# Aedelon/ProteinBERT-PyTorch-Replication

Hardware: AMD Instinct MI355X
Metric: sequences/sec (whole node) ProteinBERT pretrain L=512 at 1/2/4/8 MI355X (higher is better)
Workload: dtype bf16; 1 GPU; global_batch=2048, per_gpu_batch=2048, seq_len=512, parallelism=dp1, impl=hip, hip_graph=False

## Files before the change

### proteinbert_pytorch_replication_amd/ops/csrc/wgrad.hip

```cpp
#include "mfma.h"
#include <stdlib.h>

using namespace pbx;
typedef unsigned short bf16_t;

namespace {
constexpr int CH = 128;

constexpr int BM = 128;
constexpr int KS = 9;

__device__ __attribute__((aligned(16))) unsigned int g_zero16[4];
__device__ __attribute__((aligned(16))) unsigned int g_ones16[4] = {~0u, ~0u, ~0u, ~0u};

__device__ __forceinline__ void glds16(const void* src, unsigned char* lds_base) {
  const unsigned dst = __builtin_amdgcn_readfirstlane(
      (unsigned)(size_t)(__attribute__((address_space(3))) unsigned char*)lds_base);
  unsigned keep;
  asm volatile("s_mov_b32 %0, m0\n\ts_mov_b32 m0, %2\n\ts_nop 0\n\tglobal_load_lds_dwordx4 %1, off\n\ts_mov_b32 m0, %0"
               : "=&s"(keep)
               : "v"(src), "s"(dst)
               : "memory");
}

// ... 351 lines not shown
    sg.zero = opaque_addr(g_zero16);
    sg.ones = opaque_addr(g_ones16);
    sg.pos0 = tt0 * TBM;
    sg.L = L;
    sg.n0 = rows0 / 4;
    sg.n = rows0 / 4 + rows1 / 4;
    sg.w = w;
    sg.hal1 = hal1;
    sg.lane = lane;
    sg.lrow = lane >> 4;
    sg.lx = (unsigned)((lane & 15) ^ (((lane >> 4) & 3) << 2));
  }

  f32x16_t acc[KS];
#pragma unroll
  for (int k = 0; k < KS; ++k) acc[k] = zero16();
  const int hal = cv ? hal1 : hal0;
  const int colb = ct * 32 + tc;
  const int cvb = cv ? rows0 * 256 : 0;
  int boff[KS], boff4[KS];
#pragma unroll
  for (int k = 0; k < KS; ++k) {
    const int rb = hal + (KS / 2 - k) * d + 8 * h + q;
    boff[k] = cvb + swz256e(rb, colb);
    boff4[k] = cvb + swz256e(rb + 4, colb);
  }
  const int toff = (rows0 + rows1) * 256 + 8 * h * 8;
  if (nt > 0) {
    sg.all(smem);
    sg.next();
  }
  for (int it = 0; it < nt; ++it) {
    unsigned char* cur = smem + (it & 1) * buf_bytes;
    unsigned char* nxt = smem + ((it & 1) ^ 1) * buf_bytes;
    asm volatile("s_waitcnt vmcnt(0)" ::: "memory");
    __syncthreads();
    const int nn = it + 1 < nt ? sg.n : -1;
    constexpr int NS = (TBM / 16) * KS;
    static_assert(MAXET <= NS, "one DMA per step");
    bf16x8 fb[3], fa[2];
    unsigned tk[8];
    auto read_b = [&](int st) {
      const unsigned char* c = cur + (st / KS) * 4096;
      fb[st % 3] = cat_tr(lds_tr(c, boff[st % KS]), lds_tr(c, boff4[st % KS]));
    };
    auto read_tok = [&](int kb) {
      const unsigned* tp = reinterpret_cast<const unsigned*>(cur + toff + kb * 128);
#pragma unroll
      for (int j = 0; j < 8; ++j) tk[j] = tp[2 * j];
    };
    auto make_a = [&](int kb) {
      typedef __attribute__((ext_vector_type(4))) unsigned int u32x4;
      u32x4 o;
#pragma unroll
      for (int e = 0; e < 4; ++e)
        o[e] = (tk[2 * e] == (unsigned)r ? 0x3F80u : 0u) | (tk[2 * e + 1] == (unsigned)r ? 0x3F800000u : 0u);
      fa[kb & 1] = __builtin_bit_cast(bf16x8, o);
    };
    read_tok(0);
    make_a(0);
    read_b(0);
    read_b(1);
#pragma unroll
    for (int st = 0; st < NS; ++st) {
      const int kb = st / KS, k = st % KS;
      if (st + 2 < NS) read_b(st + 2);
      if (k == 3 && kb + 1 < TBM / 16) read_tok(kb + 1);
      if (k == 7 && kb + 1 < TBM / 16) make_a(kb + 1);
      __builtin_amdgcn_sched_barrier(0);
      if (st < MAXET) sg.issue(st, nn, nxt);
      acc[k] = mfma32(fa[kb & 1], fb[st % 3], acc[k]);
    }
    sg.next();
  }
#pragma unroll
  for (int k = 0; k < KS; ++k)
#pragma unroll
    for (int i = 0; i < 16; ++i) {
      const int v = (i & 3) + 8 * (i >> 2) + 4 * h;
      if (v < V) slab[((((size_t)blockIdx.x * 2 + cv) * KS + k) * V + v) * CH + ct * 32 + r] = acc[k][i];
    }
}

__global__ void __launch_bounds__(128) wgrad_tok_finish_kernel(const float* __restrict__ S, const float* __restrict__ E,
                                                               float* __restrict__ dw0, float* __restrict__ dw1,
                                                               float* __restrict__ db0, float* __restrict__ db1,
                                                               int V, const float* __restrict__ W0,
                                                               const float* __restrict__ W1, float* __restrict__ dEslab) {
  __shared__ float sv[KS * 32];
  const int c = blockIdx.x / CH, co = blockIdx.x % CH, ci = threadIdx.x;
  for (int i = threadIdx.x; i < KS * V; i += 128) {
    const int k = i / V, v = i % V;
    sv[k * 32 + v] = S[(((size_t)c * KS + k) * V + v) * CH + co];
  }
  __syncthreads();
  float o[KS];
#pragma unroll
  for (int k = 0; k < KS; ++k) o[k] = 0.f;
  for (int v = 0; v < V; ++v) {
    const float e = bfround(E[v * CH + ci]);
#pragma unroll
    for (int k = 0; k < KS; ++k) o[k] = fmaf(e, sv[k * 32 + v], o[k]);
  }
  float* dw = (c ? dw1 : dw0) + ((size_t)co * CH + ci) * KS;
#pragma unroll
  for (int k = 0; k < KS; ++k) dw[k] += o[k];
  if (ci == 0) {
    float s = 0.f;
    for (int v = 0; v < V; ++v) s += sv[(KS / 2) * 32 + v];
    (c ? db1 : db0)[co] += s;
  }
  if (dEslab != nullptr) {
    const float* wr = (c ? W1 : W0) + ((size_t)co * CH + ci) * KS;
    float wk[KS];
#pragma unroll
    for (int k = 0; k < KS; ++k) wk[k] = bfround(wr[k]);
    for (int v = 0; v < V; ++v) {
      float a = 0.f;
#pragma unroll
      for (int k = 0; k < KS; ++k) a = fmaf(wk[k], sv[k * 32 + v], a);
      dEslab[((size_t)blockIdx.x * V + v) * CH + ci] = a;
    }
  }
}

bool wgrad_tok_attr_set = false;
}

extern "C" int pbx_colsum_add(const float* src, int rows, int cols, float* dst, const float* scale, hipStream_t st);
extern "C" int pbx_colsum_set(const float* src, int rows, int cols, float* dst, const float* scale, hipStream_t st);

PBX_EXPORT int pbx_wgrad_tok_rows(int B, int L) {
  constexpr int cap = 256;
  const long NT = (long)B * ((L + TBM - 1) / TBM);
  return (int)(NT < cap ? NT : cap);
}

PBX_EXPORT int pbx_wgrad_tok(const void* tok, const void* dy0, const void* dy1, const float* E, float* slab, float* S,
                             float* dw0, float* dw1, float* db0, float* db1, int B, int L, int dil1, int V,
                             const float* W0, const float* W1, float* dE, float* dEslab, hipStream_t st) {
  if (V < 1 || V > 32 || dil1 < 1 || (L & 1) || B < 1 || L < 1) return (int)hipErrorInvalidValue;
  if ((dE == nullptr) != (W0 == nullptr) || (dE == nullptr) != (W1 == nullptr) || (dE == nullptr) != (dEslab == nullptr))
    return (int)hipErrorInvalidValue;
  const int buf = (2 * TBM + 8 + 8 * dil1) * 256 + 1024;
  if (2 * buf > 163840) return (int)hipErrorInvalidValue;
  if (!wgrad_tok_attr_set) {
    (void)hipFuncSetAttribute((const void*)wgrad_tok_kernel, hipFuncAttributeMaxDynamicSharedMemorySize, 163840);
    wgrad_tok_attr_set = true;
  }
  const int R = pbx_wgrad_tok_rows(B, L);
  hipLaunchKernelGGL(wgrad_tok_kernel, dim3(R), dim3(512), 2 * buf, st, (const long long*)tok, (const bf16_t*)dy0,
                     (const bf16_t*)dy1, slab, B, L, dil1, R, V, buf);
  const int cols = 2 * KS * V * CH;
  int rc = pbx_colsum_set(slab, R, cols, S, nullptr, st);
  if (rc != 0) return rc;
  hipLaunchKernelGGL(wgrad_tok_finish_kernel, dim3(2 * CH), dim3(128), 0, st, S, E, dw0, dw1, db0, db1, V, W0, W1,
                     dEslab);
  if (dE == nullptr) return pbx_launch_status();
  rc = pbx_launch_status();
  if (rc != 0) return rc;
  return pbx_colsum_add(dEslab, 2 * CH, V * CH, dE, nullptr, st);
}
```

### proteinbert_pytorch_replication_amd/ops/local_track.py

```python
from __future__ import annotations

import os
from typing import List, Dict, Optional, Tuple

import torch

from . import _lib, streams
from ..train.arena import notify_grads_ready
from ..utils.determinism import fused_deterministic
from .global_track import bf16_of

CH = 128
PB = 32
LN_EPS = 1e-5


BM1 = 128
def attn_pool_supported(NJ: int) -> bool:
    return NJ in (256, 512)


def conv_tile(L: int) -> int:
    return BM1

# ... 81 lines not shown
        _lib.call("pbx_wgrad2x", dy0.data_ptr(), _p(dy1), x.data_ptr(), slab.data_ptr(), bslab.data_ptr(),
                  dw0.data_ptr(), _p(dw1), db0.data_ptr(), _p(db1), B, L, dil, nconv, R, xlo, xhi, _lib.stream_ptr(dev))
    else:
        _lib.call("pbx_wgrad2", dy0.data_ptr(), _p(dy1), x.data_ptr(), slab.data_ptr(), bslab.data_ptr(),
                  dw0.data_ptr(), _p(dw1), db0.data_ptr(), _p(db1), B, L, dil, nconv, R, _lib.stream_ptr(dev))
    return [slab, bslab]


WGRAD_TOK = True
EMBED_FOLD = True
EMBED_GATHER = True


CONV_TOK = os.environ.get("PBX_CONV_TOK", "1") == "1"


def conv_tok_ok(B: int, L: int, KS: int, dil: int, V: int) -> bool:
    return CONV_TOK and bool(_lib.lib().pbx_conv_fwd_tok_ok(B, L, KS, dil, V))


def conv_tok_tables(wpn: torch.Tensor, wpw: torch.Tensor, emb_b: torch.Tensor) -> torch.Tensor:
    V = emb_b.shape[0]
    tab = torch.empty((2, 2, 9, V + 1, CH // 2), dtype=torch.float32, device=emb_b.device)
    _lib.call("pbx_conv_tok_tables", wpn.data_ptr(), wpw.data_ptr(), emb_b.data_ptr(), tab.data_ptr(), V,
              _lib.stream_ptr(emb_b.device))
    return tab


def conv_fwd_first(tok, emb_b, wpn, wpw, bn, bw, gb, pre_n, pre_w, s1, KS, dil, stream, tok_tab=None):
    B, L = tok.shape
    V = emb_b.shape[0]
    if conv_tok_ok(B, L, KS, dil, V):
        T1, bm1 = L // 4, 4
        st1 = torch.empty((B, T1, 2), dtype=torch.float32, device=tok.device)
        if tok_tab is None:
            tok_tab = conv_tok_tables(wpn, wpw, emb_b)
        _lib.call("pbx_conv_fwd_tok", tok.data_ptr(), emb_b.data_ptr(), tok_tab.data_ptr(), bn.data_ptr(),
                  bw.data_ptr(), gb.data_ptr(), _p(pre_n), _p(pre_w), s1.data_ptr(), st1.data_ptr(), B, L, KS, dil, V,
                  stream)
    else:
        T1, bm1 = (L + BM1 - 1) // BM1, BM1
        st1 = torch.empty((B, T1, 2), dtype=torch.float32, device=tok.device)
        _lib.call("pbx_conv_fwd3t", tok.data_ptr(), emb_b.data_ptr(), wpn.data_ptr(), wpw.data_ptr(), bn.data_ptr(),
                  bw.data_ptr(), gb.data_ptr(), _p(pre_n), _p(pre_w), s1.data_ptr(), st1.data_ptr(), B, L, KS, dil,
                  stream)
    return st1, T1, bm1


def wgrad_tok_ok(tok: Optional[torch.Tensor], emb: Optional[torch.Tensor], L: int, KS: int) -> bool:
    return (WGRAD_TOK and tok is not None and emb is not None and KS == 9 and L % 2 == 0
            and emb.shape[0] <= 32 and emb.shape[1] == CH and tok.dtype == torch.int64 and tok.is_contiguous())


def _wgrad_tok(dy0: torch.Tensor, dy1: torch.Tensor, tok: torch.Tensor, emb: torch.Tensor, dil: int, B: int, L: int,
               outs, demb=None):
    dev = dy0.device
    V = emb.shape[0]
    R = _lib.lib().pbx_wgrad_tok_rows(B, L)
    slab = torch.empty((R, 2, 9, V, CH), dtype=torch.float32, device=dev)
    S = torch.empty((2, 9, V, CH), dtype=torch.float32, device=dev)
    e = emb.detach().float().contiguous()
    (dw0, db0), (dw1, db1) = outs
    w0 = w1 = dE = dEslab = None
    if demb is not None:
        w0, w1 = (w.detach().float().contiguous() for w in demb[:2])
        dE = demb[2]
        dEslab = torch.empty((2 * CH, V, CH), dtype=torch.float32, device=dev)
    _lib.call("pbx_wgrad_tok", tok.data_ptr(), dy0.data_ptr(), dy1.data_ptr(), e.data_ptr(), slab.data_ptr(),
              S.data_ptr(), dw0.data_ptr(), dw1.data_ptr(), db0.data_ptr(), db1.data_ptr(), B, L, dil, V,
              _p(w0), _p(w1), _p(dE), _p(dEslab), _lib.stream_ptr(dev))
    return [slab, S, e, w0, w1, dEslab]


def embed_fold_bwd(tok, emb, ds1, gdn, gdw, dpn, dpw, wn, ww, stream):
    B, L = tok.shape
    dE, direct = _grad_dst(emb, emb.shape)
    slab = None
    if fused_deterministic():
        slab = torch.empty((_lib.lib().pbx_embed_bwd_groups(B * L), emb.shape[0], CH), dtype=torch.float32,
                           device=ds1.device)
    _lib.call("pbx_embed_dpre", tok.data_ptr(), ds1.data_ptr(), gdn.data_ptr(), gdw.data_ptr(), dpn.data_ptr(),
              dpw.data_ptr(), dE.data_ptr(), B * L, emb.shape[0], _p(slab), stream)
    return (wn, ww, dE), direct


class LocalBlockFn(torch.autograd.Function):

    @staticmethod
    def forward(ctx, x, gb, wn, bn, ww, bw, g1, be1, wl, bl, g2, be2, wv_bf16, dil: int, packed=None,
                tail: bool = False, cp=None, tok=None, emb=None, emb_grad: bool = False, tok_tab=None):
        params = (wn, bn, ww, bw, g1, be1, wl, bl, g2, be2)
        ctx.cp = cp
        if cp is not None:
            g1, be1, g2, be2 = (cp.rows(t) for t in (g1, be1, g2, be2))
        if x is None:
            if not (emb_grad and tok is not None and emb is not None and cp is None):
                raise ValueError("x may be None only for the folded first block (emb_grad with tok / emb)")
            B, L = tok.shape
            xt = torch.empty((B, L, CH), dtype=torch.bfloat16, device=tok.device)
        else:
            B, L, C = x.shape
            assert C == CH and x.dtype == torch.bfloat16 and x.is_contiguous()
            xt = x
        NJ = wv_bf16.shape[0]
        if not attn_pool_supported(NJ):
            raise NotImplementedError(f"HIP attention pool: H * value_dim = {NJ} (kernels built for 256 / 512)")
        KS = wn.shape[2]
        dev = xt.device
        stream = _lib.stream_ptr(dev)
        T1, bm1 = (L + BM1 - 1) // BM1, BM1
        T2 = (L + PB - 1) // PB
        if packed is not None:
            wpn, wtn, wpw, wtw = packed
        else:
            wpn, wtn = pack_conv(wn)
            wpw, wtw = pack_conv(ww)
        wl_b = bf16_of(wl)
        need_bwd = any(ctx.needs_input_grad)
        pre_n = torch.empty_like(xt) if need_bwd else None
        pre_w = torch.empty_like(xt) if need_bwd else None
        s1 = torch.empty_like(xt)
        gb = gb.detach().float().contiguous()
        from_tok = x is None or (cp is None and tok is not None and emb is not None and tok.dtype == torch.int64
                                 and tok.is_contiguous() and tuple(tok.shape) == (B, L) and emb.shape[1] == CH
                                 and conv_tok_ok(B, L, KS, dil, emb.shape[0]))
        if from_tok:
            x_ext, hlo = x, 0
            emb_b = bf16_of(emb)
            st1, T1, bm1 = conv_fwd_first(tok, emb_b, wpn, wpw, bn, bw, gb, pre_n, pre_w, s1, KS, dil, stream,
                                          tok_tab)
        elif cp is None:
            x_ext, hlo = x, 0
            st1 = torch.empty((B, T1, 2), dtype=torch.float32, device=dev)
            conv_fwd(x, wpn, wpw, bn, bw, gb, pre_n, pre_w, s1, st1, B, L, KS, dil, stream)
        else:
            x_ext, hlo = cp.halo_rows(x), cp.halo
            st1 = torch.empty((B, T1, 2), dtype=torch.float32, device=dev)
            conv_fwd(x_ext, wpn, wpw, bn, bw, gb, pre_n, pre_w, s1, st1, B, L, KS, dil, stream, hlo, hlo)
            cp.fix_stats(st1, BM1)
        pre_l = torch.empty_like(xt) if need_bwd else None
        s2 = torch.empty_like(xt)
        st2 = torch.empty((B, T2, 2), dtype=torch.float32, device=dev)
        _lib.call("pbx_ln_linear_fwd", s1.data_ptr(), st1.data_ptr(), T1, bm1, g1.data_ptr(), be1.data_ptr(),
                  wl_b.data_ptr(), bl.data_ptr(), _p(pre_l), s2.data_ptr(), st2.data_ptr(), B, L, LN_EPS, stream)
        if cp is not None:
            cp.fix_stats(st2, PB)
        h2 = torch.empty_like(xt)
        TV = (L + 31) // 32
        vpart = torch.empty((B, TV, NJ), dtype=torch.float32, device=dev)
        _lib.call("pbx_pool_fwd", s2.data_ptr(), st2.data_ptr(), g2.data_ptr(), be2.data_ptr(), wv_bf16.data_ptr(),
                  h2.data_ptr(), vpart.data_ptr(), B, L, NJ, LN_EPS, stream)
        ctx.save_for_backward(x_ext, pre_n, pre_w, s1, st1, pre_l, s2, st2, h2, wtn, wtw, wl_b, wv_bf16, g1, be1, g2,
                              be2)
        ctx.hlo = hlo
        ctx.tok = (tok, emb) if cp is None and wgrad_tok_ok(tok, emb, L, KS) else None
        ctx.emb_grad = bool(emb_grad)
        if ctx.emb_grad and (ctx.tok is None or (x is not None and x.requires_grad)):
            raise ValueError("emb_grad needs a token-embedding input without autograd history (wgrad_tok_ok)")
        ctx.meta = (B, L, KS, dil, T1, T2, NJ)
        ctx.bm1 = bm1
        ctx.tail = bool(tail) and WGRAD_TAIL_FULL
        ctx.set_materialize_grads(False)
        ctx.params = params
        return h2, vpart

    @staticmethod
    def backward(ctx, dh2, dvpart):
        streams.wait_ready(dvpart, dh2)
        (x_ext, pre_n, pre_w, s1, st1, pre_l, s2, st2, h2, wtn, wtw, wl_b, wv_bf16, g1, be1, g2,
         be2) = ctx.saved_tensors
        cp, hlo = ctx.cp, ctx.hlo
        x = s1
        B, L, KS, dil, T1, T2, NJ = ctx.meta
        bm1 = ctx.bm1
        dev = x.device
        stream = _lib.stream_ptr(dev)
        params = ctx.params
        dsts = [_grad_dst(p, p.shape) for p in params]
        (dwn, _), (dbn, _), (dww, _), (dbw, _), (dg1, _), (dbe1, _), (dwl, _), (dbl, _), (dg2, _), (dbe2, _) = dsts
        if cp is not None:
            dg1, dbe1, dg2, dbe2 = (cp.rows(t) for t in (dg1, dbe1, dg2, dbe2))
        dh2 = None if dh2 is None else dh2.to(torch.bfloat16).contiguous()
        TA = (L + 31) // 32
        if dvpart is None:
            dv, dv_tiles = torch.zeros((B, NJ), dtype=torch.float32, device=dev), 1
        elif dvpart.dim() == 3 and (dvpart.shape[1] == 1 or dvpart.stride(1) == 0):
            dv, dv_tiles = dvpart[:, 0, :].float().contiguous(), 1
        else:
            dv, dv_tiles = dvpart.float().contiguous(), TA
        dh2t = torch.empty_like(x)
        sums2 = torch.empty((B, TA, 2), dtype=torch.float32, device=dev)
        consts = torch.empty((B, 8), dtype=torch.float32, device=dev)
        dgb = torch.empty((B, CH), dtype=torch.float32, device=dev)
        _lib.call("pbx_pool_bwd", h2.data_ptr(), g2.data_ptr(), be2.data_ptr(), _p(dh2), dv.data_ptr(), dv_tiles,
                  wv_bf16.data_ptr(), dh2t.data_ptr(), sums2.data_ptr(), B, L, NJ, stream)
        if cp is not None:
            cp.fix_sums(sums2)
        dh1 = torch.empty_like(x)
        TS1 = (L + 1) // 2
        sums1 = torch.empty((B, TS1, 2), dtype=torch.float32, device=dev)
        det = int(fused_deterministic())
        late_fold = LN2_LATE_FOLD and streams.ENABLED and dev.type == "cuda" and dsts[6][1] and dsts[7][1]
        if late_fold:
            rows = _lib.lib().pbx_ln2_bwd_slab_rows(B, L, det)
            fslab = torch.empty(rows * (CH * CH + CH), dtype=torch.float32, device=dev)
            slab_args = (fslab.data_ptr(), rows)
        else:
            slab_args = dwl_slab(dev)
        _lib.call("pbx_ln2_linear_bwd", dh2t.data_ptr(), s2.data_ptr(), st2.data_ptr(), sums2.data_ptr(), TA,
                  g2.data_ptr(), pre_l.data_ptr(), s1.data_ptr(), st1.data_ptr(), T1, bm1, g1.data_ptr(),
                  be1.data_ptr(), wl_b.data_ptr(), consts.data_ptr(), dh1.data_ptr(), sums1.data_ptr(),
                  dg2.data_ptr(), dbe2.data_ptr(), dg1.data_ptr(), dbe1.data_ptr(), dwl.data_ptr(), dbl.data_ptr(),
                  dgb.data_ptr(), B, L, LN_EPS, *slab_args, det, int(not late_fold), 0, stream)
        if late_fold:
            def fold(slab=fslab, rows=rows, dwl=dwl, dbl=dbl):
                st = _lib.stream_ptr(dev)
                _lib.call("pbx_colsum_add2", slab.data_ptr(), CH * CH, dwl.data_ptr(), slab[rows * CH * CH:].data_ptr(),
                          CH, dbl.data_ptr(), rows, st)
            streams.launch(dev, fold, keep=[fslab], name="wgrad")
        dx = None if ctx.emb_grad else torch.empty_like(x)
        dpn = torch.empty_like(x)
        dpw = torch.empty_like(x)
        if cp is not None:
            cp.fix_sums(sums1)
        fin = (DGRAD_FIN and cp is None and not ctx.emb_grad and KS == 9 and dev.type == "cuda"
               and not fused_deterministic())

        def dgb_ready():
            if ctx.tail and INPUT_BWD_EARLY and streams.ENABLED and dev.type == "cuda":
                streams.fork(dev, "ann")

        if not fin:
            ds1 = torch.empty_like(x)
            _lib.call("pbx_ln1_finalize", dh1.data_ptr(), s1.data_ptr(), st1.data_ptr(), T1, bm1, sums1.data_ptr(),
                      TS1, g1.data_ptr(), ds1.data_ptr(), dgb.data_ptr(), B, L, LN_EPS, int(fused_deterministic()),
                      stream)
            if cp is not None:
                cp.all_reduce_(dgb)
            dgb_ready()
        demb = None
        if fin:
            conv_dgrad_fin(dh1, s1, st1, T1, bm1, sums1, TS1, g1, pre_n, pre_w, wtn, wtw, dx, dpn, dpw, dgb, B, L,
                           KS, dil, stream)
            dgb_ready()
        elif ctx.emb_grad:
            demb, dE_direct = embed_fold_bwd(*ctx.tok, ds1, pre_n, pre_w, dpn, dpw, params[0], params[2], stream)
            dE = demb[2]
        elif cp is None:
            conv_dgrad(ds1, pre_n, pre_w, wtn, wtw, dx, dpn, dpw, B, L, KS, dil, stream)
        else:
            conv_dgrad(*cp.halo_rows_many(ds1, pre_n, pre_w), wtn, wtw, dx, dpn, dpw, B, L,
                       KS, dil, stream, hlo, hlo)
        if ctx.tok is not None:
            tok, emb = ctx.tok
            wg = lambda: _wgrad_tok(dpn, dpw, tok, emb, dil, B, L, [(dwn, dbn), (dww, dbw)], demb)
            keep = [dpn, dpw, tok] + ([demb[2]] if demb is not None else [])
        else:
            wg = lambda: _wgrad(dpn, dpw, x_ext, KS, dil, 2, B, L, [(dwn, dbn), (dww, dbw)],
                                ctx.tail and streams.ENABLED, hlo, hlo)
            keep = [dpn, dpw, x_ext]
        direct = [p for p, (_, d) in zip(params, dsts) if d]
        if demb is not None and dE_direct:
            direct.append(ctx.tok[1])
        if all(dsts[i][1] for i in (0, 1, 2, 3)) and (demb is None or dE_direct) and streams.ENABLED:
            streams.launch(dev, wg, keep=keep, name="wgrad")
        else:
            wg()
        if direct:
            notify_grads_ready(direct)
        pgrads = [None if d else g for (g, d) in dsts]
        gemb = dE if demb is not None and not dE_direct else None
        return (dx, dgb, *pgrads, None, None, None, None, None, None, gemb, None, None)


def embed_tokens(tokens: torch.Tensor, weight: torch.Tensor) -> torch.Tensor:
    B, L = tokens.shape
    tok = tokens.contiguous()
    out = torch.empty((B, L, weight.shape[1]), dtype=torch.bfloat16, device=tokens.device)
    _lib.call("pbx_embed_fwd", tok.data_ptr(), weight.detach().contiguous().data_ptr(), out.data_ptr(), B * L,
              _lib.stream_ptr(tokens.device))
    return out


class EmbedFn(torch.autograd.Function):

    @staticmethod
    def forward(ctx, tokens, weight):
        B, L = tokens.shape
        V, C = weight.shape
        assert C == CH and V <= 32
        tok = tokens.contiguous()
        out = torch.empty((B, L, C), dtype=torch.bfloat16, device=tokens.device)
        _lib.call("pbx_embed_fwd", tok.data_ptr(), weight.detach().contiguous().data_ptr(), out.data_ptr(), B * L,
                  _lib.stream_ptr(tokens.device))
        ctx.save_for_backward(tok)
        ctx.V = V
        return out

    @staticmethod
    def backward(ctx, dout):
        (tok,) = ctx.saved_tensors
        dE = torch.zeros((ctx.V, CH), dtype=torch.float32, device=tok.device)
        d = dout.to(torch.bfloat16).contiguous()
        slab = None
        if fused_deterministic():
            g = _lib.lib().pbx_embed_bwd_groups(tok.numel())
            slab = torch.empty((g, ctx.V, CH), dtype=torch.float32, device=tok.device)
        _lib.call("pbx_embed_bwd", tok.data_ptr(), d.data_ptr(), dE.data_ptr(), tok.numel(), ctx.V, _lib.ptr(slab),
                  _lib.stream_ptr(tok.device))
        return None, dE


def _wv_bf16(att) -> torch.Tensor:
    Wv = att.Wv
    if isinstance(Wv, torch.nn.Parameter) and Wv.requires_grad:
        return att.value_weight_cat().t().to(torch.bfloat16).contiguous()
    key = (Wv.data_ptr(), Wv._version, Wv.device)
    cached = getattr(att, "_pbx_wv_cache", None)
    if cached is None or cached[0] != key:
        cached = (key, att.value_weight_cat().t().to(torch.bfloat16).contiguous())
        att._pbx_wv_cache = cached
    return cached[1]


def conv_images(wn: torch.Tensor, ww: torch.Tensor):
    KS = wn.shape[2]
    imgs = tuple(torch.empty((KS, CH, CH), dtype=torch.bfloat16, device=wn.device) for _ in range(4))
    return imgs, [(0, wn.detach(), imgs[0], imgs[1], KS, 0), (0, ww.detach(), imgs[2], imgs[3], KS, 0)]


def local_block(x: torch.Tensor, gb: torch.Tensor, blk, packed=None, tail: bool = False,
                cp=None, tok=None, emb=None, emb_grad: bool = False, tok_tab=None) -> Tuple[torch.Tensor, torch.Tensor]:
    att = blk.global_attention_layer
    wv = _wv_bf16(att)
    nc = blk.local_narrow_conv_layer[0]
    wc = blk.local_wide_conv_layer[0]
# ... 5 lines not shown
```

### proteinbert_pytorch_replication_amd/ops/paper_track.py

```python
from __future__ import annotations

import math

import torch

from . import _lib, streams
from ..train.arena import notify_grads_ready
from .gemm import gemm as _gemm
from .global_track import (BF16, F32, _Grads, _UNIT_LOSS_GRAD, bf16_of, go_head_backward, go_head_forward,
                           loss_total, mm32, addmm_into)
from .local_track import (CH, conv_dgrad, conv_fwd, conv_tile, dwl_slab, pack_conv, _grad_dst, _wgrad,
                          _wgrad_tok, embed_fold_bwd, wgrad_tok_ok)


def group_colsum(t: torch.Tensor) -> torch.Tensor:
    G, R, C = t.shape
    if t.device.type != "cuda":
        return t.sum(dim=1)
    t = t.contiguous()
    out = torch.empty((G, C), dtype=F32, device=t.device)
    _lib.call("pbx_group_colsum", t.data_ptr(), G, R, C, out.data_ptr(), _lib.stream_ptr(t.device))
    return out


def _sg_ws(B: int, G: int, H: int, K: int, dev) -> torch.Tensor:
    return torch.empty(_lib.lib().pbx_sg_query_ws(B, G, H, K), dtype=torch.float32, device=dev)

PAPER_ATTN = "fused"
FUSED_CHUNK_F = 256
FUSED_BWD_WAVES = 8

LN_EPS = 1e-5
TR = 32


class PaperBlockFn(torch.autograd.Function):

    @staticmethod
    def forward(ctx, x, gb, g, wn, bn, ww, bw, g1, be1, wl, bl, g2, be2, Wq, Wk, Wv, mask, dil: int, packed=None,
                tok=None, emb=None, emb_grad: bool = False, cp=None):
        from .paper_attention import KEY_DIM, VALUE_DIM, _nsplit
        params = (wn, bn, ww, bw, g1, be1, wl, bl, g2, be2, Wq, Wk, Wv)
        B, L, C = x.shape
        assert C == CH and x.dtype == BF16 and x.is_contiguous()
        assert g1.shape == (CH,), "paper semantics: LayerNorm affine is [C]"
        H, _, K = Wk.shape
        VD = Wv.shape[2]
        assert K == KEY_DIM and VD == VALUE_DIM
        KS = wn.shape[2]
        dev = x.device
        stream = _lib.stream_ptr(dev)
        BM1 = conv_tile(L)
        T1 = (L + BM1 - 1) // BM1
        if packed is not None:
            wpn, wtn, wpw, wtw = packed
        else:
            wpn, wtn = pack_conv(wn)
            wpw, wtw = pack_conv(ww)
        wl_b = bf16_of(wl)
        gb = gb.detach().float().contiguous()
        pre_n, pre_w, s1 = torch.empty_like(x), torch.empty_like(x), torch.empty_like(x)
        st1 = torch.empty((B, T1, 2), dtype=F32, device=dev)
        x_ext, hlo = (x, 0) if cp is None else (cp.halo_rows(x), cp.halo)
        if cp is not None and (tok is not None or emb_grad):
            raise ValueError("context parallelism: the token-embedding first-block forms are single-shard only")
        conv_fwd(x_ext, wpn, wpw, bn, bw, gb, pre_n, pre_w, s1, st1, B, L, KS, dil, stream, hlo, hlo)
        h2 = torch.empty_like(x)
        stats = torch.empty((B * L, 4), dtype=F32, device=dev)
        _lib.call("pbx_pc_ln_linear_fwd", s1.data_ptr(), g1.data_ptr(), be1.data_ptr(), wl_b.data_ptr(),
                  bl.data_ptr(), g2.data_ptr(), be2.data_ptr(), h2.data_ptr(), stats.data_ptr(), B, L, LN_EPS, stream)
        gf = g.detach().float().contiguous()
        wq32 = Wq.detach().float().contiguous()
        G = gf.shape[1]
        q = torch.empty((B, H, K), dtype=F32, device=dev)
        qs = torch.empty((B, H, K), dtype=F32, device=dev)
        _lib.call("pbx_sg_query_fwd", gf.data_ptr(), wq32.data_ptr(), q.data_ptr(), qs.data_ptr(),
                  _sg_ws(B, G, H, K, dev).data_ptr(), B, G, H, K, 1.0 / math.sqrt(K), stream)
        o = torch.empty(B, H * VD, device=dev, dtype=F32)
        lse = torch.empty(B * H, device=dev, dtype=F32)
        mk = None if mask is None else mask.contiguous()
        fused = PAPER_ATTN == "fused" and H in (2, 4)
        if fused:
            wimg = torch.empty((H, K + VD, C), dtype=BF16, device=dev)
            _lib.call("pbx_pa_wimg", Wk.detach().float().contiguous().data_ptr(),
                      Wv.detach().float().contiguous().data_ptr(), wimg.data_ptr(), H, C, K, VD, stream)
            ns = -(-L // FUSED_CHUNK_F)
            part = torch.empty(B * H, ns, 2 + VD, device=dev, dtype=F32)
            _lib.call("pbx_pa_fused_fwd", h2.data_ptr(), wimg.data_ptr(), qs.data_ptr(), _lib.ptr(mk),
                      part.data_ptr(), o.data_ptr(), lse.data_ptr(), B, L, H, stream)
            wsave, pre = wimg, None
        else:
            wcat = torch.cat([Wk.detach().permute(1, 0, 2).reshape(C, H * K),
                              Wv.detach().permute(1, 0, 2).reshape(C, H * VD)], dim=1).to(BF16)
            pre = mm32(h2.view(B * L, C), wcat).to(BF16)
            ns = _nsplit(B, H, L)
# ... 10 lines not shown
            raise ValueError("emb_grad needs a token-embedding input without autograd history (wgrad_tok_ok)")
        ctx.save_for_backward(x_ext, pre_n, pre_w, s1, stats, wtn, wtw, wl_b, q, qs, wsave, pre, mk, o, lse,
                              h2, wq32, gf)
        ctx.cp, ctx.hlo = cp, hlo
        ctx.meta = (B, L, KS, dil, BM1, H, K, VD, ns)
        ctx.params = params
        ctx.set_materialize_grads(False)
        return h2, o

    @staticmethod
    def backward(ctx, dh2, do):
        (x_ext, pre_n, pre_w, s1, stats, wtn, wtw, wl_b, q, qs, wsave, pre, mk, o, lse, h2,
         wq32, gf32) = ctx.saved_tensors
        B, L, KS, dil, BM1, H, K, VD, ns = ctx.meta
        cp, hlo = ctx.cp, ctx.hlo
        x = x_ext if cp is None else x_ext[:, hlo:hlo + L]
        dev = x.device
        stream = _lib.stream_ptr(dev)
        params = ctx.params
        wn, bn, ww, bw, g1, be1, wl, bl, g2, be2, Wq, Wk, Wv = params
        dsts = [_grad_dst(p, p.shape) for p in params]
        (dwn, _), (dbn, _), (dww, _), (dbw, _), (dg1, _), (dbe1, _), (dwl, _), (dbl, _), (dg2, _), (dbe2, _) = dsts[:10]
        (dWq, _), (dWk, _), (dWv, _) = dsts[10:]
        R, C = B * L, CH
        dh2 = None if dh2 is None else dh2.to(BF16).contiguous()
        dg = None
        dh2_att = [None, None]
        if do is not None:
            dO = do.float().contiguous()
            if ctx.fused:
                npair = H // 2
                dh2p = torch.empty((npair, B, L, C), dtype=BF16, device=dev)
                dpre = torch.empty((R, H * (K + VD)), dtype=BF16, device=dev)
                nsb = -(-L // (32 * FUSED_BWD_WAVES))
                dq_part = torch.empty(B * H, nsb, K, device=dev, dtype=F32)
                _lib.call("pbx_pa_fused_bwd", h2.data_ptr(), wsave.data_ptr(), qs.data_ptr(), _lib.ptr(mk),
                          lse.data_ptr(), o.data_ptr(), dO.data_ptr(), dh2p.data_ptr(), dpre.data_ptr(),
                          dq_part.data_ptr(), B, L, H, FUSED_BWD_WAVES, stream)
                dh2_att = [dh2p[i] for i in range(npair)] + [None] * (2 - npair)
            else:
                dpre = torch.empty_like(pre)
                dq_part = torch.empty(B * H, ns, K, device=dev, dtype=F32)
                _lib.call("pbx_paper_attn_bwd", pre.data_ptr(), qs.data_ptr(), _lib.ptr(mk), lse.data_ptr(),
                          o.data_ptr(), dO.data_ptr(), dpre.data_ptr(), dq_part.data_ptr(), B, L, H, K, VD, ns,
                          stream)
                dh2_att = [mm32(dpre, wsave.t()).to(BF16), None]
            dqs = group_colsum(dq_part).view(B, H, K)
            if cp is not None:
                cp.all_reduce_(dqs)
            G = gf32.shape[1]
            dg = torch.empty((B, G), dtype=F32, device=dev)
            _lib.call("pbx_sg_query_dg", dqs.data_ptr(), q.data_ptr(), wq32.data_ptr(), dg.data_ptr(),
                      _sg_ws(B, G, H, K, dev).data_ptr(), B, G, H, K, 1.0 / math.sqrt(K), stream)

            def att_wgrad(dpre=dpre, h2=h2, dqs=dqs, q=q, gf32=gf32):
                dwcat = torch.empty((C, dpre.shape[1]), dtype=F32, device=dev)
                _gemm(h2.reshape(R, C), dpre, dwcat, ta=True, tb=False)
                if dWk.is_contiguous() and dWv.is_contiguous():
                    _lib.call("pbx_pa_dwkv_add", dwcat.data_ptr(), dWk.data_ptr(), dWv.data_ptr(), H, C, K, VD,
                              _lib.stream_ptr(dev))
                else:
                    dWk.add_(dwcat[:, :H * K].view(C, H, K).permute(1, 0, 2))
                    dWv.add_(dwcat[:, H * K:].view(C, H, VD).permute(1, 0, 2))
                ws = _sg_ws(B, G, H, K, dev)
                _lib.call("pbx_sg_query_dwq", gf32.data_ptr(), dqs.data_ptr(), q.data_ptr(), dWq.data_ptr(),
                          ws.data_ptr(), B, G, H, K, 1.0 / math.sqrt(K), _lib.stream_ptr(dev))
                return [dwcat, ws]

            if streams.ENABLED and dev.type == "cuda" and all(d for _, d in dsts[10:]):
                streams.launch(dev, att_wgrad, keep=[dpre, h2, dqs, q, gf32], name="wgrad")
            else:
                att_wgrad()
        ds1 = torch.empty_like(x)
        T = (L + TR - 1) // TR
        dgbp = torch.empty((B, T, CH), dtype=F32, device=dev)
        _lib.call("pbx_pc_ln_linear_bwd", _lib.ptr(dh2), _lib.ptr(dh2_att[0]), _lib.ptr(dh2_att[1]),
                  s1.data_ptr(), stats.data_ptr(),
                  g1.data_ptr(), be1.data_ptr(), wl_b.data_ptr(), bl.data_ptr(), g2.data_ptr(), ds1.data_ptr(),
                  dgbp.data_ptr(), dg2.data_ptr(), dbe2.data_ptr(), dg1.data_ptr(), dbe1.data_ptr(), dwl.data_ptr(),
                  dbl.data_ptr(), *dwl_slab(dev), B, L, stream)
        dgb = group_colsum(dgbp)
        if cp is not None:
            cp.all_reduce_(dgb)
        dpn, dpw = torch.empty_like(x), torch.empty_like(x)
        demb, dE_direct, dx = None, True, None
        if ctx.emb_grad:
            demb, dE_direct = embed_fold_bwd(*ctx.tok, ds1, pre_n, pre_w, dpn, dpw, wn, ww, stream)
        elif cp is None:
            dx = torch.empty_like(x)
            conv_dgrad(ds1, pre_n, pre_w, wtn, wtw, dx, dpn, dpw, B, L, KS, dil, stream)
        else:
            dx = torch.empty_like(x)
            conv_dgrad(*cp.halo_rows_many(ds1, pre_n, pre_w), wtn, wtw, dx, dpn, dpw, B, L, KS, dil, stream,
                       hlo, hlo)
        if ctx.tok is not None:
            tok, emb = ctx.tok
            wg = lambda: _wgrad_tok(dpn, dpw, tok, emb, dil, B, L, [(dwn, dbn), (dww, dbw)], demb)
        else:
            wg = lambda: _wgrad(dpn, dpw, x_ext, KS, dil, 2, B, L, [(dwn, dbn), (dww, dbw)],
                                xlo=hlo, xhi=hlo)
        if all(dsts[i][1] for i in (0, 1, 2, 3)) and dE_direct and streams.ENABLED:
            streams.launch(dev, wg, keep=[dpn, dpw, x_ext] + ([demb[2]] if demb is not None else []), name="wgrad")
        else:
            wg()
        direct = [p for p, (_, d) in zip(params, dsts) if d]
        if demb is not None and dE_direct:
            direct.append(ctx.tok[1])
        if direct:
            notify_grads_ready(direct)
        pgrads = [None if d else gr for (gr, d) in dsts]
        gemb = demb[2] if demb is not None and not dE_direct else None
        return (dx, dgb, dg, *pgrads, None, None, None, None, gemb, None, None)


def _cp_softmax_combine(o: torch.Tensor, lse: torch.Tensor, B: int, H: int, VD: int, cp):
    import torch.distributed as dist
    empty = torch.isposinf(lse)
    lr = torch.where(empty, torch.full_like(lse, -float("inf")), lse)
    m = lr.clone()
    dist.all_reduce(m, op=dist.ReduceOp.MAX, group=cp.group)
    mz = torch.where(torch.isfinite(m), m, torch.zeros_like(m))
    w = torch.exp(lr - mz)
    ow = torch.where(w[:, None] > 0, o.view(B * H, VD) * w[:, None], torch.zeros_like(o.view(B * H, VD)))
    s = torch.cat([w, ow.reshape(-1)])
    dist.all_reduce(s, group=cp.group)
    sw = s[:B * H]
    has = sw > 0
    o_g = torch.where(has[:, None], s[B * H:].view(B * H, VD) / sw.clamp_min(1e-30)[:, None], 0.0)
    lse_g = torch.where(has, mz + torch.log(sw.clamp_min(1e-30)), torch.full_like(sw, float("inf")))
    return o_g.reshape(B, H * VD).contiguous(), lse_g.contiguous()


def paper_block(x: torch.Tensor, gb: torch.Tensor, g: torch.Tensor, blk, mask, packed=None, tok=None, emb=None,
                emb_grad: bool = False, cp=None):
    nc = blk.local_narrow_conv_layer[0]
    wc = blk.local_wide_conv_layer[0]
    att = blk.global_attention_layer
    return PaperBlockFn.apply(x, gb, g, nc.weight, nc.bias, wc.weight, wc.bias, blk.local_norm_1.weight,
                              blk.local_norm_1.bias, blk.local_linear_layer[0].weight,
                              blk.local_linear_layer[0].bias, blk.local_norm_2.weight, blk.local_norm_2.bias,
                              att.Wq, att.Wk, att.Wv, mask, blk.wide_conv_dilation, packed, tok, emb, emb_grad, cp)


def paper_local_block(x: torch.Tensor, gb: torch.Tensor, blk, packed=None) -> torch.Tensor:
    g = torch.zeros((x.shape[0], blk.global_dim), dtype=F32, device=x.device)
    h2, _ = paper_block(x, gb, g, blk, None, packed)
    return h2


_ONES = {}


def unit_attention_weight(K: int, device) -> torch.Tensor:
    key = (K, str(device))
    t = _ONES.get(key)
    if t is None:
        t = torch.ones(K, dtype=F32, device=device)
        _ONES[key] = t
    return t


class PaperHeadsLossFn(torch.autograd.Function):

    @staticmethod
    def forward(ctx, h, g2, g2_bf, wo, bo, wa, ba, y_l, y_g, w_l, w_g):
        dev = h.device
        st = _lib.stream_ptr(dev)
        B, L, C = h.shape
        V = wo.shape[0]
        A = wa.shape[0]
        loss = torch.empty(2, dtype=F32, device=dev)
        R = B * L
        hb = h.reshape(R, C)
        parts = _lib.lib().pbx_paper_head_parts(R)
        dh = torch.empty((B, L, C), dtype=BF16, device=dev)
        dzl = torch.empty((R, 32), dtype=BF16, device=dev)
        dbo_part = torch.empty((parts, V), dtype=F32, device=dev)
        loss_part = torch.empty(parts, dtype=F32, device=dev)
        y = y_l.reshape(-1).contiguous()
        wl = w_l.reshape(-1).float().contiguous()
        _lib.call("pbx_paper_head", hb.data_ptr(), wo.detach().float().contiguous().data_ptr(),
                  bo.detach().float().contiguous().data_ptr(), y.data_ptr(), wl.data_ptr(), dh.data_ptr(),
                  dzl.data_ptr(), dbo_part.data_ptr(), loss_part.data_ptr(), R, V, 1.0 / float(R), st)
        _lib.call("pbx_colsum_set", loss_part.data_ptr(), parts, 1, loss.data_ptr(), None, st)
        dbo = torch.empty(V, dtype=F32, device=dev)
# ... 31 lines not shown
```

Baseline: 112,800 sequences/s.

## Fuse embedding-fold dpre products into token weight-gradient kernel

For the first (embedding-folded) block, the separate embed_dpre pass that wrote dpn/dpw tensors is skipped. A new wgrad_tok_fold kernel loads ds1, gdn and gdw tiles into LDS, forms the gated products in place, and runs the one-hot token MFMA weight-gradient. It also accumulates an extra residual term for the embedding gradient, which the finish kernel copies into an extra dEslab row. This removes two full-size intermediate activations and one kernel pass, at the cost of smaller tiles (64 rows), extra LDS work and a larger slab reduction.

Result: no change. 113,300 sequences/s, median of 6 (+0.5%).

```diff
diff --git a/proteinbert_pytorch_replication_amd/ops/csrc/wgrad.hip b/proteinbert_pytorch_replication_amd/ops/csrc/wgrad.hip
--- a/proteinbert_pytorch_replication_amd/ops/csrc/wgrad.hip
+++ b/proteinbert_pytorch_replication_amd/ops/csrc/wgrad.hip
@@ -457,12 +457,20 @@
     }
 }
 
+template <bool RES>
 __global__ void __launch_bounds__(128) wgrad_tok_finish_kernel(const float* __restrict__ S, const float* __restrict__ E,
                                                                float* __restrict__ dw0, float* __restrict__ dw1,
                                                                float* __restrict__ db0, float* __restrict__ db1,
                                                                int V, const float* __restrict__ W0,
                                                                const float* __restrict__ W1, float* __restrict__ dEslab) {
   __shared__ float sv[KS * 32];
+  if constexpr (RES) {
+    if (blockIdx.x == 2 * CH) {
+      for (int i = threadIdx.x; i < V * CH; i += 128)
+        dEslab[(size_t)2 * CH * V * CH + i] = S[(size_t)2 * KS * V * CH + i];
+      return;
+    }
+  }
   const int c = blockIdx.x / CH, co = blockIdx.x % CH, ci = threadIdx.x;
   for (int i = threadIdx.x; i < KS * V; i += 128) {
     const int k = i / V, v = i % V;
@@ -529,10 +537,244 @@
   const int cols = 2 * KS * V * CH;
   int rc = pbx_colsum_set(slab, R, cols, S, nullptr, st);
   if (rc != 0) return rc;
-  hipLaunchKernelGGL(wgrad_tok_finish_kernel, dim3(2 * CH), dim3(128), 0, st, S, E, dw0, dw1, db0, db1, V, W0, W1,
-                     dEslab);
+  hipLaunchKernelGGL(wgrad_tok_finish_kernel<false>, dim3(2 * CH), dim3(128), 0, st, S, E, dw0, dw1, db0, db1, V, W0,
+                     W1, dEslab);
   if (dE == nullptr) return pbx_launch_status();
   rc = pbx_launch_status();
   if (rc != 0) return rc;
   return pbx_colsum_add(dEslab, 2 * CH, V * CH, dE, nullptr, st);
 }
+
+namespace {
+constexpr int FBM = 64;
+constexpr int FNR = FBM + 2 * (KS / 2);
+constexpr int MAXEF = 10;
+
+struct StageFold {
+  unsigned long db, wb, nb, tokb;
+  unsigned long dys, toks;
+  unsigned long zero, ones;
+  int pos0, L, Lp;
+  int nw, n, w;
+  int hal1;
+  int lane0;
+
+  __device__ __forceinline__ void issue(int e, int nn, unsigned char* buf, int lane) const {
+    const int i = w + 8 * e;
+    if (i > nn) return;
+    const int lrow = lane >> 4;
+    const unsigned lx = (unsigned)((lane & 15) ^ ((lrow & 3) << 2));
+    if (i == n) {
+      const int p = pos0 + 2 * lane;
+      unsigned long a = tokb + (unsigned long)(unsigned)p * 8u;
+      asm volatile("" : "+v"(a));
+      glds16((const void*)(lane < 32 && p < L ? a : ones), buf + n * 1024);
+      return;
+    }
+    const int img = i < nw ? 0 : i < 2 * nw ? 1 : 2;
+    const int j = i - img * nw;
+    const int r0 = pos0 - (img == 2 ? KS / 2 : hal1) + 4 * j;
+    const unsigned lo = (unsigned)(lrow * 256) + ((lx ^ (unsigned)(j & 3)) << 4);
+    unsigned long a = (img == 0 ? db : img == 1 ? wb : nb) + (unsigned long)((long)r0 * 256) + lo;
+    asm volatile("" : "+v"(a));
+    glds16((const void*)((unsigned)(r0 + lrow) < (unsigned)L ? a : zero), buf + i * 1024);
+  }
+  __device__ __forceinline__ void all(int nn, unsigned char* buf) const {
+    int lane = lane0;
+    asm volatile("" : "+v"(lane));
+#pragma unroll
+    for (int e = 0; e < MAXEF; ++e) issue(e, nn, buf, lane);
+  }
+  __device__ __forceinline__ void next() {
+    pos0 += FBM;
+    if (pos0 >= Lp) {
+      pos0 = 0;
+      db += dys;
+      wb += dys;
+      nb += dys;
+      tokb += toks;
+    }
+  }
+};
+
+template <bool RES>
+__device__ __forceinline__ void fold_tiles(unsigned char* smem, int buf_bytes, int nt, StageFold& sg,
+                                           f32x16_t (&acc)[KS], f32x16_t& accr, int rowsw, int d, int cv, int ct,
+                                           int lane, int tid) {
+  const int r = lane & 31, h = lane >> 5;
+  const int q = tr_q(lane), tc = tr_c(lane);
+  const int hal1 = sg.hal1;
+  const int hal = cv ? hal1 : KS / 2;
+  const int colb = ct * 32 + tc;
+  constexpr int NB = KS + (RES ? 1 : 0);
+  const int cvb = (cv ? rowsw : 2 * rowsw) * 256;
+  int boff[NB], boff4[NB];
+#pragma unroll
+  for (int k = 0; k < NB; ++k) {
+    const int rb = (k < KS ? hal + (KS / 2 - k) * d : hal1) + 8 * h + q;
+    const int base = k < KS ? cvb : 0;
+    boff[k] = base + swz256e(rb, colb);
+    boff4[k] = base + swz256e(rb + 4, colb);
+  }
+  const int toff = (2 * rowsw + FNR) * 256 + 8 * h * 8;
+  if (nt > 0) {
+    sg.all(sg.n, smem);
+    sg.next();
+  }
+  for (int it = 0; it < nt; ++it) {
+    unsigned char* cur = smem + (it & 1) * buf_bytes;
+    unsigned char* nxt = smem + ((it & 1) ^ 1) * buf_bytes;
+    asm volatile("s_waitcnt vmcnt(0)" ::: "memory");
+    __syncthreads();
+    if (it + 1 < nt) {
+      sg.all(sg.n, nxt);
+      sg.next();
+    }
+    for (int idx = tid; idx < rowsw * 16; idx += 512) {
+      const int row = idx >> 4, c = idx & 15;
+      const int o = swz256(row, c);
+      float g[8], p[8], y[8];
+      unpack8(*reinterpret_cast<const uint4*>(cur + o), g);
+      uint4* pw = reinterpret_cast<uint4*>(cur + rowsw * 256 + o);
+      unpack8(*pw, p);
+#pragma unroll
+      for (int e = 0; e < 8; ++e) y[e] = p[e] * g[e];
+      *pw = packq8(y);
+      const int rn = row - (hal1 - KS / 2);
+      if ((unsigned)rn < (unsigned)FNR) {
+        uint4* pn = reinterpret_cast<uint4*>(cur + 2 * rowsw * 256 + swz256(rn, c));
+        unpack8(*pn, p);
+#pragma unroll
+        for (int e = 0; e < 8; ++e) y[e] = p[e] * g[e];
+        *pn = packq8(y);
+      }
+    }
+    __syncthreads();
+    constexpr int NS = (FBM / 16) * NB;
+    bf16x8 fb[3], fa[2];
+    unsigned tk[8];
+    auto read_b = [&](int st) {
+      const unsigned char* c = cur + (st / NB) * 4096;
+      fb[st % 3] = cat_tr(lds_tr(c, boff[st % NB]), lds_tr(c, boff4[st % NB]));
+    };
+    auto read_tok = [&](int kb) {
+      const unsigned* tp = reinterpret_cast<const unsigned*>(cur + toff + kb * 128);
+#pragma unroll
+      for (int j = 0; j < 8; ++j) tk[j] = tp[2 * j];
+    };
+    auto make_a = [&](int kb) {
+      typedef __attribute__((ext_vector_type(4))) unsigned int u32x4;
+      u32x4 o;
+#pragma unroll
+      for (int e = 0; e < 4; ++e)
+        o[e] = (tk[2 * e] == (unsigned)r ? 0x3F80u : 0u) | (tk[2 * e + 1] == (unsigned)r ? 0x3F800000u : 0u);
+      fa[kb & 1] = __builtin_bit_cast(bf16x8, o);
+    };
+    read_tok(0);
+    make_a(0);
+    read_b(0);
+    read_b(1);
+#pragma unroll
+    for (int st = 0; st < NS; ++st) {
+      const int kb = st / NB, k = st % NB;
+      if (st + 2 < NS) read_b(st + 2);
+      if (k == 3 && kb + 1 < FBM / 16) read_tok(kb + 1);
+      if (k == 7 && kb + 1 < FBM / 16) make_a(kb + 1);
+      __builtin_amdgcn_sched_barrier(0);
+      if (k < KS)
+        acc[k] = mfma32(fa[kb & 1], fb[st % 3], acc[k]);
+      else
+        accr = mfma32(fa[kb & 1], fb[st % 3], accr);
+    }
+  }
+}
+
+__global__ void __launch_bounds__(512, 1) wgrad_tok_fold_kernel(const long long* __restrict__ tok,
+                                                                const bf16_t* __restrict__ ds1,
+                                                                const bf16_t* __restrict__ gdn,
+                                                                const bf16_t* __restrict__ gdw,
+                                                                float* __restrict__ slab, int B, int L, int dil1,
+                                                                int R, int V, int buf_bytes) {
+  extern __shared__ __attribute__((aligned(16))) unsigned char smem[];
+  const int tid = threadIdx.x, lane = tid & 63, w = __builtin_amdgcn_readfirstlane(tid >> 6);
+  const int r = lane & 31, h = lane >> 5;
+  const int cv = w >> 2, ct = w & 3;
+  const int hal1 = (KS / 2) * dil1;
+  const int rowsw = FBM + 2 * hal1;
+  const int T = (L + TBM - 1) / TBM;
+  const long NT = (long)B * T;
+  const long t0 = NT * blockIdx.x / R, t1 = NT * (blockIdx.x + 1) / R;
+  const int nt = (int)(t1 - t0) * (TBM / FBM);
+
+  StageFold sg;
+  {
+    const int b0 = (int)(t0 / T), tt0 = (int)(t0 - (long)b0 * T);
+    sg.dys = (unsigned long)L * CH * 2;
+    sg.toks = (unsigned long)L * 8;
+    sg.db = (unsigned long)ds1 + (unsigned long)b0 * sg.dys;
+    sg.wb = (unsigned long)gdw + (unsigned long)b0 * sg.dys;
+    sg.nb = (unsigned long)gdn + (unsigned long)b0 * sg.dys;
+    sg.tokb = (unsigned long)tok + (unsigned long)b0 * sg.toks;
+    sg.zero = opaque_addr(g_zero16);
+    sg.ones = opaque_addr(g_ones16);
+    sg.pos0 = tt0 * TBM;
+    sg.L = L;
+    sg.Lp = T * TBM;
+    sg.nw = rowsw / 4;
+    sg.n = 2 * (rowsw / 4) + FNR / 4;
+    sg.w = w;
+    sg.hal1 = hal1;
+    sg.lane0 = lane;
+  }
+
+  f32x16_t acc[KS], accr = zero16();
+#pragma unroll
+  for (int k = 0; k < KS; ++k) acc[k] = zero16();
+  if (cv == 0)
+    fold_tiles<true>(smem, buf_bytes, nt, sg, acc, accr, rowsw, 1, 0, ct, lane, tid);
+  else
+    fold_tiles<false>(smem, buf_bytes, nt, sg, acc, accr, rowsw, dil1, 1, ct, lane, tid);
+  float* dst = slab + (size_t)blockIdx.x * (2 * KS + 1) * V * CH + ct * 32 + r;
+#pragma unroll
+  for (int k = 0; k < KS; ++k)
+#pragma unroll
+    for (int i = 0; i < 16; ++i) {
+      const int v = (i & 3) + 8 * (i >> 2) + 4 * h;
+      if (v < V) dst[((size_t)(cv * KS + k) * V + v) * CH] = acc[k][i];
+    }
+  if (cv == 0) {
+#pragma unroll
+    for (int i = 0; i < 16; ++i) {
+      const int v = (i & 3) + 8 * (i >> 2) + 4 * h;
+      if (v < V) dst[((size_t)(2 * KS) * V + v) * CH] = accr[i];
+    }
+  }
+}
+
+bool wgrad_tok_fold_attr_set = false;
+}
+
+PBX_EXPORT int pbx_wgrad_tok_fold(const void* tok, const void* ds1, const void* gdn, const void* gdw, const float* E,
+                                  const float* W0, const float* W1, float* slab, float* S, float* dEslab, float* dw0,
+                                  float* dw1, float* db0, float* db1, float* dE, int B, int L, int dil1, int V,
+                                  hipStream_t st) {
+  if (V < 1 || V > 32 || dil1 < 1 || (L & 1) || B < 1 || L < 1) return (int)hipErrorInvalidValue;
+  if (dE == nullptr || W0 == nullptr || W1 == nullptr || dEslab == nullptr) return (int)hipErrorInvalidValue;
+  if (dil1 > 7) return (int)hipErrorInvalidValue;
+  const int buf = (2 * (FBM + 8 * dil1) + FNR) * 256 + 1024;
+  if (2 * buf > 163840 || (2 * (FBM + 8 * dil1) + FNR) / 4 + 1 > 8 * MAXEF) return (int)hipErrorInvalidValue;
+  if (!wgrad_tok_fold_attr_set) {
+    (void)hipFuncSetAttribute((const void*)wgrad_tok_fold_kernel, hipFuncAttributeMaxDynamicSharedMemorySize, 163840);
+    wgrad_tok_fold_attr_set = true;
+  }
+  const int R = pbx_wgrad_tok_rows(B, L);
+  hipLaunchKernelGGL(wgrad_tok_fold_kernel, dim3(R), dim3(512), 2 * buf, st, (const long long*)tok, (const bf16_t*)ds1,
+                     (const bf16_t*)gdn, (const bf16_t*)gdw, slab, B, L, dil1, R, V, buf);
+  int rc = pbx_colsum_set(slab, R, (2 * KS + 1) * V * CH, S, nullptr, st);
+  if (rc != 0) return rc;
+  hipLaunchKernelGGL(wgrad_tok_finish_kernel<true>, dim3(2 * CH + 1), dim3(128), 0, st, S, E, dw0, dw1, db0, db1, V, W0,
+                     W1, dEslab);
+  rc = pbx_launch_status();
+  if (rc != 0) return rc;
+  return pbx_colsum_add(dEslab, 2 * CH + 1, V * CH, dE, nullptr, st);
+}
diff --git a/proteinbert_pytorch_replication_amd/ops/local_track.py b/proteinbert_pytorch_replication_amd/ops/local_track.py
--- a/proteinbert_pytorch_replication_amd/ops/local_track.py
+++ b/proteinbert_pytorch_replication_amd/ops/local_track.py
@@ -187,6 +187,30 @@
     _lib.call("pbx_embed_dpre", tok.data_ptr(), ds1.data_ptr(), gdn.data_ptr(), gdw.data_ptr(), dpn.data_ptr(),
               dpw.data_ptr(), dE.data_ptr(), B * L, emb.shape[0], _p(slab), stream)
     return (wn, ww, dE), direct
+
+
+EMBED_FOLD_FUSED = os.environ.get("PBX_EMBED_FOLD_FUSED", "1") == "1"
+
+
+def embed_fold_fused_ok(dil: int) -> bool:
+    return EMBED_FOLD_FUSED and 1 <= dil <= 7
+
+
+def _wgrad_tok_fold(ds1: torch.Tensor, gdn: torch.Tensor, gdw: torch.Tensor, tok: torch.Tensor, emb: torch.Tensor,
+                    dil: int, B: int, L: int, outs, wn: torch.Tensor, ww: torch.Tensor, dE: torch.Tensor):
+    dev = ds1.device
+    V = emb.shape[0]
+    R = _lib.lib().pbx_wgrad_tok_rows(B, L)
+    slab = torch.empty((R, 19, V, CH), dtype=torch.float32, device=dev)
+    S = torch.empty((19, V, CH), dtype=torch.float32, device=dev)
+    dEslab = torch.empty((2 * CH + 1, V, CH), dtype=torch.float32, device=dev)
+    e = emb.detach().float().contiguous()
+    w0, w1 = (w.detach().float().contiguous() for w in (wn, ww))
+    (dw0, db0), (dw1, db1) = outs
+    _lib.call("pbx_wgrad_tok_fold", tok.data_ptr(), ds1.data_ptr(), gdn.data_ptr(), gdw.data_ptr(), e.data_ptr(),
+              w0.data_ptr(), w1.data_ptr(), slab.data_ptr(), S.data_ptr(), dEslab.data_ptr(), dw0.data_ptr(),
+              dw1.data_ptr(), db0.data_ptr(), db1.data_ptr(), dE.data_ptr(), B, L, dil, V, _lib.stream_ptr(dev))
+    return [slab, S, dEslab, e, w0, w1]
 
 
 class LocalBlockFn(torch.autograd.Function):
@@ -324,8 +348,9 @@
                           CH, dbl.data_ptr(), rows, st)
             streams.launch(dev, fold, keep=[fslab], name="wgrad")
         dx = None if ctx.emb_grad else torch.empty_like(x)
-        dpn = torch.empty_like(x)
-        dpw = torch.empty_like(x)
+        fused = ctx.emb_grad and embed_fold_fused_ok(dil)
+        dpn = None if fused else torch.empty_like(x)
+        dpw = None if fused else torch.empty_like(x)
         if cp is not None:
             cp.fix_sums(sums1)
         fin = (DGRAD_FIN and cp is None and not ctx.emb_grad and KS == 9 and dev.type == "cuda"
@@ -348,6 +373,9 @@
             conv_dgrad_fin(dh1, s1, st1, T1, bm1, sums1, TS1, g1, pre_n, pre_w, wtn, wtw, dx, dpn, dpw, dgb, B, L,
                            KS, dil, stream)
             dgb_ready()
+        elif fused:
+            dE, dE_direct = _grad_dst(ctx.tok[1], ctx.tok[1].shape)
+            demb = (params[0], params[2], dE)
         elif ctx.emb_grad:
             demb, dE_direct = embed_fold_bwd(*ctx.tok, ds1, pre_n, pre_w, dpn, dpw, params[0], params[2], stream)
             dE = demb[2]
@@ -356,7 +384,12 @@
         else:
             conv_dgrad(*cp.halo_rows_many(ds1, pre_n, pre_w), wtn, wtw, dx, dpn, dpw, B, L,
                        KS, dil, stream, hlo, hlo)
-        if ctx.tok is not None:
+        if fused:
+            tok, emb = ctx.tok
+            wg = lambda: _wgrad_tok_fold(ds1, pre_n, pre_w, tok, emb, dil, B, L,
+                                         [(dwn, dbn), (dww, dbw)], *demb)
+            keep = [ds1, pre_n, pre_w, tok, dE]
+        elif ctx.tok is not None:
             tok, emb = ctx.tok
             wg = lambda: _wgrad_tok(dpn, dpw, tok, emb, dil, B, L, [(dwn, dbn), (dww, dbw)], demb)
             keep = [dpn, dpw, tok] + ([demb[2]] if demb is not None else [])
diff --git a/proteinbert_pytorch_replication_amd/ops/paper_track.py b/proteinbert_pytorch_replication_amd/ops/paper_track.py
--- a/proteinbert_pytorch_replication_amd/ops/paper_track.py
+++ b/proteinbert_pytorch_replication_amd/ops/paper_track.py
@@ -10,7 +10,7 @@
 from .global_track import (BF16, F32, _Grads, _UNIT_LOSS_GRAD, bf16_of, go_head_backward, go_head_forward,
                            loss_total, mm32, addmm_into)
 from .local_track import (CH, conv_dgrad, conv_fwd, conv_tile, dwl_slab, pack_conv, _grad_dst, _wgrad,
-                          _wgrad_tok, embed_fold_bwd, wgrad_tok_ok)
+                          _wgrad_tok, _wgrad_tok_fold, embed_fold_bwd, embed_fold_fused_ok, wgrad_tok_ok)
 
 
 def group_colsum(t: torch.Tensor) -> torch.Tensor:
@@ -187,9 +187,13 @@
         dgb = group_colsum(dgbp)
         if cp is not None:
             cp.all_reduce_(dgb)
-        dpn, dpw = torch.empty_like(x), torch.empty_like(x)
+        fused = ctx.emb_grad and embed_fold_fused_ok(dil)
+        dpn, dpw = (None, None) if fused else (torch.empty_like(x), torch.empty_like(x))
         demb, dE_direct, dx = None, True, None
-        if ctx.emb_grad:
+        if fused:
+            dE, dE_direct = _grad_dst(ctx.tok[1], ctx.tok[1].shape)
+            demb = (wn, ww, dE)
+        elif ctx.emb_grad:
             demb, dE_direct = embed_fold_bwd(*ctx.tok, ds1, pre_n, pre_w, dpn, dpw, wn, ww, stream)
         elif cp is None:
             dx = torch.empty_like(x)
@@ -198,14 +202,21 @@
             dx = torch.empty_like(x)
             conv_dgrad(*cp.halo_rows_many(ds1, pre_n, pre_w), wtn, wtw, dx, dpn, dpw, B, L, KS, dil, stream,
                        hlo, hlo)
-        if ctx.tok is not None:
+        if fused:
+            tok, emb = ctx.tok
+            wg = lambda: _wgrad_tok_fold(ds1, pre_n, pre_w, tok, emb, dil, B, L,
+                                         [(dwn, dbn), (dww, dbw)], *demb)
+            keep = [ds1, pre_n, pre_w, tok, demb[2]]
+        elif ctx.tok is not None:
             tok, emb = ctx.tok
             wg = lambda: _wgrad_tok(dpn, dpw, tok, emb, dil, B, L, [(dwn, dbn), (dww, dbw)], demb)
+            keep = [dpn, dpw, x_ext] + ([demb[2]] if demb is not None else [])
         else:
             wg = lambda: _wgrad(dpn, dpw, x_ext, KS, dil, 2, B, L, [(dwn, dbn), (dww, dbw)],
                                 xlo=hlo, xhi=hlo)
+            keep = [dpn, dpw, x_ext]
         if all(dsts[i][1] for i in (0, 1, 2, 3)) and dE_direct and streams.ENABLED:
-            streams.launch(dev, wg, keep=[dpn, dpw, x_ext] + ([demb[2]] if demb is not None else []), name="wgrad")
+            streams.launch(dev, wg, keep=keep, name="wgrad")
         else:
             wg()
         direct = [p for p, (_, d) in zip(params, dsts) if d]
```
